# cherubicXN/neat

Hardware: AMD Instinct MI355X
Metric: ray-samples/s (train step) on ABC-neat-a (higher is better)
Workload: dtype bf16; 1 GPU; C2: abc-neat-a networks, 1024 rays x 128 samples per GPU, depth samples given, train step = forward + loss + backward + Adam; rays_per_gpu=1024, samples_per_ray=128, global_rays=1024, parallelism=dp1, weights=synthetic 'rough' (seed 42), launch=hip graph replay, the whole step one launch (forward + loss + backward + Adam)

## Files before the change

include/neat_hip.h:

```cpp
#ifndef NEAT_HIP_H
#define NEAT_HIP_H
#include <stddef.h>
#ifdef __cplusplus
extern "C" {
#endif

#define NEAT_NUM_LAYERS 19
#define NEAT_FEATURE 256

typedef struct neat_net_params {
  const float* v[NEAT_NUM_LAYERS];
  const float* g[NEAT_NUM_LAYERS];
  const float* b[NEAT_NUM_LAYERS];
} neat_net_params;

typedef struct neat_net_grads {
  float* dv[NEAT_NUM_LAYERS];
  float* dg[NEAT_NUM_LAYERS];
  float* db[NEAT_NUM_LAYERS];
} neat_net_grads;

int neat_abi_version(void);

#define NEAT_F32 0
// ... 129 lines not shown
int neat_project2d_pair(const float* K, const float* K2, const float* w2c, const float* X, int N, float* uv, float* uv2, void* stream);
int neat_line_loss(const float* pred, const float* gt, const float* weight, int R, float threshold, float* out2, float* per_line,
                   float* d_pred, void* stream);
int neat_line_losses(const float* pred_px, const float* pred_calib, const float* gt5, const float* K, int R, float threshold, float* out3,
                     float* d_pred_calib, float grad_scale, void* stream);

int neat_adam_step(float* params, const float* const* grads, const long long* seg_offsets, const int* seg_steps, int nseg,
                   float* exp_avg, float* exp_avg_sq, float lr, float beta1, float beta2, float eps, void* stream);
int neat_adam_step_coef(float* params, const float* const* grads, const long long* seg_offsets, int nseg, float* exp_avg, float* exp_avg_sq,
                        const float* coef, float beta1, float beta2, float eps, void* stream);

size_t neat_lsap_ws_bytes(int nr, int nc);
int neat_lsap(const float* cost, int nr, int nc, const unsigned char* row_mask, const unsigned char* col_mask, long long* row_ind,
              long long* col_ind, int* n_match, void* ws, void* stream);

size_t neat_dbscan_ws_bytes(int n);
int neat_dbscan_means(const float* points, int n, double eps, float* centres, unsigned char* valid, int* count, void* ws, void* stream);

int neat_parse_match(const float* lines2d, int n, const float* gt, int m, int gt_stride, float threshold, int* label, float* mindis,
                     void* stream);
size_t neat_parse_group_ws_bytes(int n, int m);
int neat_parse_group(const int* label, const float* lines3d, const float* l3d, int n, int m, float* lines, float* scores, int* count,
                     void* ws, void* stream);
size_t neat_parse_vote_ws_bytes(int J, int mcap);
int neat_parse_vote(const float* junctions, int J, const float* lines, const int* count, int mcap, float threshold, int view, int* votes,
                    int* first, void* ws, void* stream);
size_t neat_parse_graph_ws_bytes(int V, int mcap, int J);
int neat_parse_graph(const float* vlines, const float* vscores, const int* vcount, int V, int mcap, float score_threshold,
                     const float* junctions, const int* votes, const int* first, int J, float* lines_out, float* junc_out,
                     unsigned char* graph, int* pairs, float* wfi, int ecap, int* counts, void* ws, void* stream);
// ... 23 lines not shown
```

neat_amd/_lib.py:

```python
import ctypes
import os

NUM_LAYERS = 19
ABI_VERSION = 15
PRECISIONS = {"fp32": 0, "bf16": 1, "bf16x3": 2, "fp16": 3, "fp16x3": 4}
_HERE = os.path.dirname(os.path.abspath(__file__))
LIB_PATH = os.environ.get("NEAT_HIP_LIB") or os.path.join(_HERE, "csrc", "libneat_hip.so")

c_fp = ctypes.c_void_p


class NetParams(ctypes.Structure):
    _fields_ = [("v", c_fp * NUM_LAYERS), ("g", c_fp * NUM_LAYERS), ("b", c_fp * NUM_LAYERS)]


class NetGrads(ctypes.Structure):
    _fields_ = [("dv", c_fp * NUM_LAYERS), ("dg", c_fp * NUM_LAYERS), ("db", c_fp * NUM_LAYERS)]


_SIGNATURES = {
    "neat_abi_version": (ctypes.c_int, []),
    "neat_packed_floats": (ctypes.c_size_t, [ctypes.c_int]),
    "neat_pack_weights": (ctypes.c_int, [ctypes.POINTER(NetParams), c_fp, ctypes.c_int, c_fp]),
    "neat_eik_points": (ctypes.c_int, [c_fp, c_fp, c_fp, c_fp, c_fp, ctypes.c_int, ctypes.c_int, c_fp, c_fp, ctypes.c_int, c_fp, c_fp]),
# ... 65 lines not shown
                                          c_fp, c_fp, c_fp]),
    "neat_loss_terms": (ctypes.c_int, [c_fp, c_fp, ctypes.c_int, c_fp, ctypes.c_int, c_fp, c_fp, ctypes.c_int, c_fp, c_fp, ctypes.c_int,
                                       c_fp, c_fp, c_fp, c_fp, ctypes.c_float, c_fp]),
    "neat_loss_pairs": (ctypes.c_int, [c_fp, c_fp, c_fp, ctypes.c_int, c_fp, c_fp, c_fp, c_fp, c_fp, c_fp, ctypes.c_int, c_fp, c_fp, c_fp,
                                       c_fp, c_fp, ctypes.c_float, ctypes.c_float, ctypes.c_float, ctypes.c_float, ctypes.c_int, c_fp, c_fp, c_fp]),
    "neat_camera_mats": (ctypes.c_int, [c_fp, c_fp, ctypes.c_int, c_fp, c_fp, c_fp]),
    "neat_inv_small": (ctypes.c_int, [c_fp, ctypes.c_int, ctypes.c_int, c_fp, c_fp]),
    "neat_project2d": (ctypes.c_int, [c_fp, c_fp, c_fp, ctypes.c_int, c_fp, c_fp]),
    "neat_project2d_backward": (ctypes.c_int, [c_fp, c_fp, c_fp, ctypes.c_int, c_fp, c_fp, c_fp]),
    "neat_line_loss": (ctypes.c_int, [c_fp, c_fp, c_fp, ctypes.c_int, ctypes.c_float, c_fp, c_fp, c_fp, c_fp]),
    "neat_line_losses": (ctypes.c_int, [c_fp, c_fp, c_fp, c_fp, ctypes.c_int, ctypes.c_float, c_fp, c_fp, ctypes.c_float, c_fp]),
    "neat_adam_step": (ctypes.c_int, [c_fp, ctypes.POINTER(ctypes.c_void_p), ctypes.POINTER(ctypes.c_longlong), ctypes.POINTER(ctypes.c_int),
                                      ctypes.c_int, c_fp, c_fp, ctypes.c_float, ctypes.c_float, ctypes.c_float, ctypes.c_float, c_fp]),
    "neat_lsap_ws_bytes": (ctypes.c_size_t, [ctypes.c_int, ctypes.c_int]),
    "neat_lsap": (ctypes.c_int, [c_fp, ctypes.c_int, ctypes.c_int, c_fp, c_fp, c_fp, c_fp, c_fp, c_fp, c_fp]),
    "neat_dbscan_ws_bytes": (ctypes.c_size_t, [ctypes.c_int]),
    "neat_dbscan_means": (ctypes.c_int, [c_fp, ctypes.c_int, ctypes.c_double, c_fp, c_fp, c_fp, c_fp, c_fp]),
    "neat_parse_match": (ctypes.c_int, [c_fp, ctypes.c_int, c_fp, ctypes.c_int, ctypes.c_int, ctypes.c_float, c_fp, c_fp, c_fp]),
    "neat_parse_group_ws_bytes": (ctypes.c_size_t, [ctypes.c_int, ctypes.c_int]),
    "neat_parse_group": (ctypes.c_int, [c_fp, c_fp, c_fp, ctypes.c_int, ctypes.c_int, c_fp, c_fp, c_fp, c_fp, c_fp]),
    "neat_parse_vote_ws_bytes": (ctypes.c_size_t, [ctypes.c_int, ctypes.c_int]),
    "neat_parse_vote": (ctypes.c_int, [c_fp, ctypes.c_int, c_fp, c_fp, ctypes.c_int, ctypes.c_float, ctypes.c_int, c_fp, c_fp, c_fp, c_fp]),
    "neat_parse_graph_ws_bytes": (ctypes.c_size_t, [ctypes.c_int, ctypes.c_int, ctypes.c_int]),
    "neat_parse_graph": (ctypes.c_int, [c_fp, c_fp, c_fp, ctypes.c_int, ctypes.c_int, ctypes.c_float, c_fp, c_fp, c_fp, ctypes.c_int,
                                        c_fp, c_fp, c_fp, c_fp, c_fp, ctypes.c_int, c_fp, c_fp, c_fp]),
    "neat_parse_visibility_ws_bytes": (ctypes.c_size_t, [ctypes.c_int, ctypes.c_int]),
    "neat_parse_visibility": (ctypes.c_int, [c_fp, c_fp, ctypes.c_int, c_fp, ctypes.c_int, c_fp, c_fp, c_fp, ctypes.c_int, ctypes.c_float,
                                             ctypes.c_int, c_fp, c_fp, c_fp, c_fp, c_fp]),
    "neat_grid_points": (ctypes.c_int, [c_fp, ctypes.c_int, ctypes.c_longlong, ctypes.c_int, ctypes.POINTER(ctypes.c_int),
                                        ctypes.POINTER(ctypes.c_double), ctypes.POINTER(ctypes.c_double), c_fp]),
# ... 51 lines not shown
```

neat_amd/csrc/kernels_junction.hpp:

```cpp
#pragma once
#include <hip/hip_runtime.h>
#include "device_util.hpp"

namespace neat {

constexpr int LSAP_WG = 1024;

struct LsapArgs {
  const float* cost;
  int nr, nc;
  const unsigned char* row_mask;
  long long* row_ind;
  long long* col_ind;
  int* n_match;
  double* wsd;
  int* wsi;
  int use_lds, lds_int_off;
  const unsigned char* col_mask;
  int cost_lds_off;
};

struct LsapKey { double val; int it; int un; };

__device__ __forceinline__ bool lsap_better(const LsapKey& a, const LsapKey& b) {
// ... 1016 lines not shown
}

struct LossPairsArgs {
  const long long* ri; const long long* ci; const int* n_match; int Kmax;
  const float* loc3; const float* loc2c; const float* loc2;
  const float* glo3; const float* glo2c; const float* glo2; int J;
  const float* pair_cost;
  float* scal;
  float* d_glo3; float* d_glo2c;
  const float* line_loss; float w_eik, w_line, w_j3, w_j2;
  int weighted_grads;
  float* total;
  const float* w2c;
};

__global__ __launch_bounds__(1024) void loss_pairs_kernel(LossPairsArgs a) {
  __shared__ float s_red[16];
  const int tid = threadIdx.x, nt = blockDim.x;
  for (int i = tid; i < 3 * a.J; i += nt) a.d_glo3[i] = 0.0f;
  for (int i = tid; i < 2 * a.J; i += nt) a.d_glo2c[i] = 0.0f;
  __syncthreads();
  const int n = max(*a.n_match, 0);
  const float inv = 1.0f / (float)max(n, 1);
  const float g3 = a.weighted_grads ? a.w_j3 : 1.0f, g2 = a.weighted_grads ? a.w_j2 : 1.0f;
  float s3 = 0.0f, s2 = 0.0f, spx = 0.0f, cnt = 0.0f;
  for (int q = tid; q < a.Kmax; q += nt) {
    const long long r = a.ri[q], c = a.ci[q];
    if (r < 0 || c < 0 || q >= n) continue;
#pragma unroll
    for (int e = 0; e < 3; ++e) {
      const float d = a.loc3[3 * r + e] - a.glo3[3 * c + e];
// ... 15 lines not shown
      const float x[3] = {a.glo3[3 * j], a.glo3[3 * j + 1], a.glo3[3 * j + 2]};
      float dX[3];
      project_bwd_calib(a.w2c, x, a.d_glo2c[2 * j], a.d_glo2c[2 * j + 1], dX);
#pragma unroll
      for (int e = 0; e < 3; ++e) a.d_glo3[3 * j + e] += dX[e];
    }
  }
  if (tid == 0) {
    a.scal[2] = s3 * inv; a.scal[3] = s2 * inv; a.scal[4] = spx * inv; a.scal[5] = cnt;
    const float tot = a.scal[0] + a.w_eik * a.scal[1] + a.w_line * a.line_loss[0] + a.w_j3 * (s3 * inv) + a.w_j2 * (s2 * inv);
    a.scal[6] = tot;
    if (a.total) a.total[0] = tot;
  }
}

__global__ void l3d_kernel(const float* __restrict__ x, const float* __restrict__ o, const float* __restrict__ d,
                           const float* __restrict__ nrm, int R, float* __restrict__ l3d) {
  const int r = blockIdx.x * blockDim.x + threadIdx.x;
  if (r >= R) return;
  float den = 0.0f, num = 0.0f;
#pragma unroll
  for (int c = 0; c < 3; ++c) { den += d[3 * r + c] * nrm[3 * r + c]; num += (x[3 * r + c] - o[3 * r + c]) * nrm[3 * r + c]; }
  den += den >= 0.0f ? 1e-6f : -1e-6f;
  const float t = num / den;
#pragma unroll
  for (int c = 0; c < 3; ++c) l3d[3 * r + c] = o[3 * r + c] + d[3 * r + c] * t;
}

__global__ void junction_cost_kernel(const float* __restrict__ cand2d, const float* __restrict__ gt2d, int V, int C, float* __restrict__ cost) {
  const int idx = blockIdx.x * blockDim.x + threadIdx.x;
  if (idx >= V * C) return;
  const int v = idx / C, c = idx % C;
  const float dx = cand2d[2 * c] - gt2d[2 * v], dy = cand2d[2 * c + 1] - gt2d[2 * v + 1];
  cost[idx] = __fsqrt_rn(__fadd_rn(__fmul_rn(dx, dx), __fmul_rn(dy, dy)));
}

struct JunctionGateArgs {
  const long long* rows; const long long* cols; int K;
  const float* cost; int C;
  const float* cand3d; const float* cand2d; const float* cand2dc;
  int use_median;
  float* median;
  unsigned char* good;
  float* j3d; float* j2d; float* j2dc;
};

__global__ __launch_bounds__(1024) void junction_gate_kernel(JunctionGateArgs a) {
  __shared__ float s_m[2048];
  __shared__ int s_n;
  __shared__ float s_med;
  const int tid = threadIdx.x, nt = blockDim.x;
  if (tid == 0) { s_n = 0; s_med = 10.0f; }
  __syncthreads();
  for (int k = tid; k < a.K; k += nt) {
    const long long r = a.rows[k], c = a.cols[k];
    const bool ok = r >= 0 && c >= 0;
    s_m[k] = ok ? a.cost[r * a.C + c] : NAN;
    if (ok) atomicAdd(&s_n, 1);
  }
  __syncthreads();
  const int n = s_n;
  if (a.use_median && n > 0) {
// ... 9 lines not shown
  __syncthreads();
  const float thr = a.use_median ? s_med : 10.0f;
  if (tid == 0 && a.use_median) a.median[0] = s_med;
  for (int k = tid; k < a.K; k += nt) {
    const float v = s_m[k];
    const bool ok = v == v;
    a.good[k] = (ok && v < thr) ? 1 : 0;
    const long long c = ok ? a.cols[k] : 0;
#pragma unroll
    for (int e = 0; e < 3; ++e) a.j3d[3 * k + e] = ok ? a.cand3d[3 * c + e] : 0.0f;
#pragma unroll
    for (int e = 0; e < 2; ++e) { a.j2d[2 * k + e] = ok ? a.cand2d[2 * c + e] : 0.0f; a.j2dc[2 * k + e] = ok ? a.cand2dc[2 * c + e] : 0.0f; }
  }
}

}
```

neat_amd/csrc/neat_aux.hip:

```cpp
#include "kernels_sampler.hpp"
#include "kernels_junction.hpp"
#include "kernels_parse.hpp"
#include "kernels_mesh.hpp"
#include "../../include/neat_hip.h"
#include <algorithm>
#include <cmath>
#include <limits.h>
#include <math.h>

using namespace neat;

__attribute__((visibility("hidden"))) int neat_aux_set_tuning(int key, int value);

namespace {

int g_ffn_mfma = 1;
int g_sampler_ablate = 0;

#define NEAT_CHECK(expr) do { hipError_t e_ = (expr); if (e_ != hipSuccess) return (int)e_; } while (0)
inline dim3 grid1(int n, int b = 256) { return dim3((n + b - 1) / b); }

__global__ void volume_weights_kernel(const float* __restrict__ z, const float* __restrict__ sdf, int R, int S,
                                      const float* __restrict__ beta_ptr, float* __restrict__ weights) {
  const float beta = *beta_ptr;
// ... 439 lines not shown
  size_t lds = 0;
  constexpr size_t LSAP_LDS_MAX = 156 * 1024;
  a.cost_lds_off = -1;
  if (dbytes + ibytes <= LSAP_LDS_MAX) {
    NEAT_CHECK(lds_limit<&lsap_kernel>((int)LSAP_LDS_MAX));
    a.use_lds = 1; a.lds_int_off = (int)dbytes; lds = (dbytes + ibytes + 15) & ~(size_t)15;
    const size_t cbytes = (size_t)nr * nc * sizeof(float);
    if (lds + cbytes <= LSAP_LDS_MAX) { a.cost_lds_off = (int)lds; lds += cbytes; }
  }
  int threads = (int)((mx + 1) / 2 + 63) / 64 * 64;
  threads = threads < 64 ? 64 : (threads > LSAP_WG ? LSAP_WG : threads);
  hipLaunchKernelGGL(lsap_kernel, dim3(1), dim3(threads), lds, (hipStream_t)stream, a);
  return (int)hipGetLastError();
}

size_t neat_dbscan_ws_bytes(int n) { return (size_t)n * 2 * sizeof(int); }

int neat_dbscan_means(const float* points, int n, double eps, float* centres, unsigned char* valid, int* count, void* ws, void* stream) {
  if (n <= 0 || n > DBSCAN_MAXN || !points || !centres || !valid || !count || !ws || !(eps > 0.0)) return -1;
  int* parent = (int*)ws; int* has_nb = parent + n;
  hipLaunchKernelGGL(dbscan_init_kernel, dim3((n + 255) / 256), dim3(256), 0, (hipStream_t)stream, parent, has_nb, n);
  hipLaunchKernelGGL(dbscan_union_kernel, dim3(n), dim3(128), 0, (hipStream_t)stream, points, n, eps * eps, parent, has_nb);
  const size_t acc_bytes = (size_t)(n / 2) * 28 + (size_t)n * 4, pbytes = (size_t)n * 12;
  const int mode = acc_bytes <= 96 * 1024 ? 2 : (pbytes <= 96 * 1024 ? 1 : 0);
  if (mode) NEAT_CHECK(lds_limit<&dbscan_finish_kernel>(96 * 1024));
  hipLaunchKernelGGL(dbscan_finish_kernel, dim3(1), dim3(1024), mode == 2 ? acc_bytes : (mode == 1 ? pbytes : 0), (hipStream_t)stream, points, n,
                     parent, has_nb, centres, valid, count, mode);
  return (int)hipGetLastError();
}

// ... 200 lines not shown
```

neat_amd/networks.py:

```python
import math

import numpy as np
import os

import torch
from torch import nn

from . import ops, rend_util
from .conf import ConfTree, from_dict
from .density import LaplaceDensity
from .ray_sampler import ErrorBoundSampler, HierarchicalSampler


def _wn_linear(in_dim, out_dim, weight_norm=True):
    lin = nn.Linear(in_dim, out_dim)
    if not weight_norm:
        raise NotImplementedError("the HIP path implements the weight-normed layers of the shipped confs")
    return lin


DEFAULT_PRECISION = "fp16x3"


def _wrap_wn(lin):
# ... 390 lines not shown
        output = {"points": points, "rgb_values": rgb, "sdf": sdf_s, "depth": depth, "xyz": xyz}

        points3d = xyz
        main = torch.cuda.current_stream() if xyz.is_cuda else None
        side = self._side_stream(xyz.device) if (main is not None and self.use_side_stream) else None
        if setup is not None:
            w2c, K3 = setup[3], setup[4]
        elif xyz.is_cuda and pose.shape[1:] == (4, 4) and intrinsics.dtype == torch.float32 and intrinsics.stride(-1) == 1:
            w2c, K3 = ops.camera_mats(pose[0], intrinsics[0])
        else:
            w2c = ops.inv_small(pose[0])[:3]
            K3 = intrinsics[0, :3, :3]
        Rm, T = w2c[:, :3], w2c[:, 3:]
        eye = _eye3(K3.device)

        def l3d_block():
            if points3d.is_cuda:
                net = self.implicit_network
                p3_sdf, p3_grad = ops.sdf_point_normals(net.handle(), points3d, net.sdf_bounding_sphere, net.sphere_scale)
            else:
                p3_sdf, _, p3_grad = self.implicit_network.get_outputs(points3d)
            l_dirs, l_orig = (setup[2], cam_loc) if setup is not None else self._rays(input, "uv_proj")
            if points3d.is_cuda:
                l3d = ops.l3d_points(points3d, l_orig, l_dirs, p3_grad)
            else:
                den = (l_dirs * p3_grad).sum(-1)
                den = den + torch.where(den >= 0, torch.full_like(den, 1e-6), torch.full_like(den, -1e-6))
                t = (((points3d - l_orig) * p3_grad).sum(-1) / den).detach()
                l3d = l_orig + l_dirs * t.unsqueeze(-1)
            l3d_score = None
            if self.training and self.use_l3d:
                with torch.no_grad():
                    a, b = l3d - lines3d[:, 0], l3d - lines3d[:, 1]
                    l3d_score = torch.linalg.cross(a, b).norm(dim=-1) / (lines3d[:, 0] - lines3d[:, 1]).norm(dim=-1)
            return p3_sdf, l3d, l3d_score

        j3d_global = None
        if side is not None:
# ... 21 lines not shown
                side_b = None
        else:
            side_b = None
            if self.training:
                j3d_global = self._global_junctions()
            p3_sdf, l3d, l3d_score = l3d_block()
        if xyz.is_cuda:
            K3c, w2c3 = K3.contiguous(), w2c.contiguous()
            K3 = K3c
            proj = lambda Kc, X: ops.project2d(Kc, w2c3, X)
            proj_pair = lambda X: ops.project2d_pair(K3c, eye, w2c3, X)
        else:
            K3c = K3
            proj = lambda Kc, X: self.project2D(Kc, Rm, T, X)
            proj_pair = lambda X: (proj(K3c, X), proj(eye, X))
        if xyz.is_cuda:
            lines2d, lines2d_calib = proj_pair(lines3d)
            lines2d = lines2d.detach()
        else:
            lines2d = proj(K3c, lines3d.detach())
            lines2d_calib = proj(eye, lines3d)
        if self.training:
            cand_valid = None
            if self.dbscan_enabled:
                if lines3d.is_cuda and 2 <= 2 * n_rays <= ops.DBSCAN_MAX_POINTS:
                    cand3d, cand_valid, _ = ops.dbscan_means(lines3d.detach().reshape(-1, 3), 0.01)
                else:
                    cand3d = self.cluster_dbscan(lines3d.detach().cpu().numpy().reshape(-1, 3), eps=0.01, min_samples=2)
            elif self.use_l3d:
                thr = l3d_score.median().clamp_min(0.01)
                keep = l3d_score < thr
                cand3d = torch.cat([lines3d[keep].detach().reshape(-1, 3), l3d[keep]], 0)
            else:
                cand3d = lines3d.detach().reshape(-1, 3)
            if self.dbscan_enabled or self.use_l3d:
                cand2d, cand2d_calib = proj_pair(cand3d)
            else:
                cand2d = lines2d.reshape(-1, 2)
                cand2d_calib = lines2d_calib.detach().reshape(-1, 2)
            gt2d = _device_copy(input["wireframe"][0], "vertices", cand2d.device)
            fused_gate = cand2d.is_cuda and min(gt2d.shape[0], cand2d.shape[0]) <= 2048
            cost = ops.junction_cost(cand2d, gt2d) if fused_gate else ((cand2d[None] - gt2d[:, None]) ** 2).sum(-1).sqrt()
            rows, cols, _ = ops.linear_sum_assignment(cost, None, cand_valid)
            if fused_gate:
                median, good, j3_pad, j2_pad, j2c_pad = ops.junction_gate(rows, cols, cost, cand3d, cand2d, cand2d_calib, self.use_median)
                if self.use_median:
                    output["median"] = median
            else:
                if cand_valid is None:
                    matched = cost[rows, cols]
                    pair_ok = None
                else:
                    pair_ok = rows >= 0
                    rows, cols = rows.clamp_min(0), cols.clamp_min(0)
                    matched = torch.where(pair_ok, cost[rows, cols], torch.full_like(cost[rows, cols], float("nan")))
# ... 85 lines not shown
```

neat_amd/ops.py:

```python
import ctypes

import torch

from . import _lib

NET_LAYOUT = (("implicit_network", 9), ("rendering_network", 5), ("attraction_network", 5))
LAYER_OUT = [256, 256, 256, 217, 256, 256, 256, 256, 257, 256, 256, 256, 256, 3, 256, 256, 256, 256, 6]
LAYER_IN = [39, 256, 256, 256, 256, 256, 256, 256, 256, 289, 256, 256, 256, 256, 265, 256, 256, 256, 256]
N_SDF = 9


def _p(t):
    return ctypes.c_void_p(t.data_ptr()) if t is not None else None


def _stream():
    return ctypes.c_void_p(torch.cuda.current_stream().cuda_stream)


def copy_batch(pairs):
    lib = _lib.lib()
    for i0 in range(0, len(pairs), 16):
        chunk = pairs[i0:i0 + 16]
        n = len(chunk)
# ... 748 lines not shown
        line3 = torch.empty(3, device=dev)
        fold = lines3d is not None and w2c is not None
        x3_c, w2c_c = (_f32c(lines3d.detach().reshape(-1, 6)), _f32c(w2c.detach())) if fold else (None, None)
        if fold and (x3_c.shape[0] != L or w2c_c.shape != (3, 4)):
            raise RuntimeError("loss_tail: lines3d [L,2,3] and w2c [3,4]")
        sizes = [R * 3, E * 3, J * 3 if have_pairs else 0, J * 2 if have_pairs else 0, L * 4, L * 6 if fold else 0]
        flat = torch.empty(sum(sizes), device=dev)
        d_rgb, d_gth, d_glo3, d_glo2c, d_pred, d_x3 = flat.split(sizes)
        d_gth = d_gth if E else None
        pair_cost = torch.empty(K, J, device=dev) if have_pairs else None
        _lib.check(lib.neat_loss_lines_terms(_p(pu), _p(pc), _p(g5), _p(Kc), L, float(threshold), _p(line3), _p(d_pred), w_line,
                                             _p(rgb_c), _p(gt_c), R, _p(gth_c), E, _p(loc3_c), _p(loc2c_c), K, _p(glo3_c), _p(glo2c_c), J,
                                             _p(scal), _p(d_rgb), _p(d_gth), _p(pair_cost), w_eik, _p(w2c_c), _p(x3_c), _p(d_x3) if fold else None,
                                             _stream()), "neat_loss_lines_terms")
        if have_pairs:
            ri, ci, n_match = linear_sum_assignment(pair_cost, good)
            loss = torch.empty((), device=dev)
            _lib.check(lib.neat_loss_pairs(_p(ri), _p(ci), _p(n_match), ri.shape[0], _p(loc3_c), _p(loc2c_c), _p(loc2_c), _p(glo3_c),
                                           _p(glo2c_c), _p(glo2_c), J, _p(pair_cost), _p(scal), _p(d_glo3), _p(d_glo2c),
                                           _ip(line3, 1), w_eik, w_line, w_j3, w_j2, 1, _p(loss), _p(w2c_c), _stream()), "neat_loss_pairs")
        else:
            loss = scal[0] + w_eik * scal[1] + w_line * line3[1]
        ctx.save_for_backward(flat)
        ctx.sizes = sizes
        ctx.set_materialize_grads(False)
        ctx.shapes = (rgb.shape, None if gtheta is None else gtheta.shape, None if glo3 is None or not have_pairs else glo3.shape,
                      None if glo2c is None or not have_pairs or fold else glo2c.shape, None if fold else pred_calib.shape,
                      lines3d.shape if fold else None)
        ctx.mark_non_differentiable(scal, line3)
        return loss, scal, line3

    @staticmethod
    def backward(ctx, g_loss, g_scal, g_line3):
        if g_loss is None:
            return (None,) * 21
# ... 124 lines not shown
    _lib.check(_lib.lib().neat_junction_cost(_p(cand2d), _p(gt2d), V, C, _p(cost), _stream()), "neat_junction_cost")
    return cost


def junction_gate(rows, cols, cost, cand3d, cand2d, cand2d_calib, use_median):
    K = rows.shape[0]
    dev = cost.device
    cand3d, cand2d, cand2d_calib = _f32c(cand3d.detach()), _f32c(cand2d.detach()), _f32c(cand2d_calib.detach())
    median = torch.empty(1, device=dev) if use_median else None
    good = torch.empty(K, device=dev, dtype=torch.uint8)
    j3d, j2d, j2dc = torch.empty(K, 3, device=dev), torch.empty(K, 2, device=dev), torch.empty(K, 2, device=dev)
    _lib.check(_lib.lib().neat_junction_gate(_p(rows), _p(cols), K, _p(cost), cost.shape[1], _p(cand3d), _p(cand2d), _p(cand2d_calib),
                                             1 if use_median else 0, _p(median), _p(good), _p(j3d), _p(j2d), _p(j2dc), _stream()),
               "neat_junction_gate")
    return (median.reshape(()) if use_median else None), good.view(torch.bool), j3d, j2d, j2dc


def _i32(t):
    if t.dtype != torch.int32 or not t.is_cuda:
        raise RuntimeError("neat_amd parse ops need CUDA int32 tensors: got %s on %s" % (t.dtype, t.device))
    return t.contiguous()


def _ws(nbytes, device):
    return torch.empty(max(int(nbytes), 8), device=device, dtype=torch.uint8)


def _rows4(gt):
    gt = _f32c(gt.detach()) if gt.stride(-1) != 1 or gt.dtype != torch.float32 or not gt.is_cuda else gt.detach()
    if gt.dim() != 2 or gt.shape[1] < 4:
# ... 118 lines not shown
```

Baseline: 49.27 million ray-samples/s.

## Fuse junction projection, cost, LSAP and gating into single-wave GPU kernels

Adds a wave-level Hungarian (LSAP) solver for small assignment problems and fuses it with the projection, cost-matrix build and junction gating into one kernel. Extra blocks of the same launch also compute l3d and the global junction projections. A second fused kernel runs the pair LSAP inside the loss-pairs kernel. The aim is to cut the chain of small kernel launches and the separate general LSAP path inside the graphed train step. In exchange it adds LDS-bound size limits and a serial single-wave solver that only covers small problem sizes.

```diff
diff --git a/include/neat_hip.h b/include/neat_hip.h
--- a/include/neat_hip.h
+++ b/include/neat_hip.h
@@ -167,6 +167,17 @@
 int neat_lsap(const float* cost, int nr, int nc, const unsigned char* row_mask, const unsigned char* col_mask, long long* row_ind,
               long long* col_ind, int* n_match, void* ws, void* stream);
 
+int neat_lsap_few_ok(int nr, int nc);
+int neat_junction_match(const float* K, const float* K2, const float* w2c, const float* cand3d, int C, const unsigned char* cand_valid,
+                        const float* gt2d, int V, int use_median, float* cand2d, float* cand2d_calib, long long* rows, long long* cols,
+                        int* n_match, float* median, unsigned char* good, float* j3d, float* j2d, float* j2d_calib, const float* l_x,
+                        const float* l_o, const float* l_d, const float* l_normal, int R, float* l3d, const float* glo3, int J, float* glo2,
+                        float* glo2_calib, void* stream);
+int neat_loss_pairs_match(const float* pair_cost, int K, int J, const unsigned char* good, long long* ri, long long* ci, int* n_match,
+                          const float* loc3, const float* loc2c, const float* loc2, const float* glo3, const float* glo2c, const float* glo2,
+                          float* scal, float* d_glo3, float* d_glo2c, const float* line_loss, float w_eik, float w_line, float w_j3, float w_j2,
+                          int weighted_grads, float* total, const float* w2c, void* stream);
+
 size_t neat_dbscan_ws_bytes(int n);
 int neat_dbscan_means(const float* points, int n, double eps, float* centres, unsigned char* valid, int* count, void* ws, void* stream);
 
diff --git a/neat_amd/_lib.py b/neat_amd/_lib.py
--- a/neat_amd/_lib.py
+++ b/neat_amd/_lib.py
@@ -103,6 +103,11 @@
                                       ctypes.c_int, c_fp, c_fp, ctypes.c_float, ctypes.c_float, ctypes.c_float, ctypes.c_float, c_fp]),
     "neat_lsap_ws_bytes": (ctypes.c_size_t, [ctypes.c_int, ctypes.c_int]),
     "neat_lsap": (ctypes.c_int, [c_fp, ctypes.c_int, ctypes.c_int, c_fp, c_fp, c_fp, c_fp, c_fp, c_fp, c_fp]),
+    "neat_lsap_few_ok": (ctypes.c_int, [ctypes.c_int, ctypes.c_int]),
+    "neat_junction_match": (ctypes.c_int, [c_fp, c_fp, c_fp, c_fp, ctypes.c_int, c_fp, c_fp, ctypes.c_int, ctypes.c_int] + [c_fp] * 14
+                            + [ctypes.c_int, c_fp, c_fp, ctypes.c_int, c_fp, c_fp, c_fp]),
+    "neat_loss_pairs_match": (ctypes.c_int, [c_fp, ctypes.c_int, ctypes.c_int] + [c_fp] * 14
+                              + [ctypes.c_float, ctypes.c_float, ctypes.c_float, ctypes.c_float, ctypes.c_int, c_fp, c_fp, c_fp]),
     "neat_dbscan_ws_bytes": (ctypes.c_size_t, [ctypes.c_int]),
     "neat_dbscan_means": (ctypes.c_int, [c_fp, ctypes.c_int, ctypes.c_double, c_fp, c_fp, c_fp, c_fp, c_fp]),
     "neat_parse_match": (ctypes.c_int, [c_fp, ctypes.c_int, c_fp, ctypes.c_int, ctypes.c_int, ctypes.c_float, c_fp, c_fp, c_fp]),
diff --git a/neat_amd/csrc/kernels_junction.hpp b/neat_amd/csrc/kernels_junction.hpp
--- a/neat_amd/csrc/kernels_junction.hpp
+++ b/neat_amd/csrc/kernels_junction.hpp
@@ -1054,7 +1054,7 @@
   const float* w2c;
 };
 
-__global__ __launch_bounds__(1024) void loss_pairs_kernel(LossPairsArgs a) {
+__device__ __forceinline__ void loss_pairs_body(const LossPairsArgs& a) {
   __shared__ float s_red[16];
   const int tid = threadIdx.x, nt = blockDim.x;
   for (int i = tid; i < 3 * a.J; i += nt) a.d_glo3[i] = 0.0f;
@@ -1100,25 +1100,38 @@
   }
 }
 
+__global__ __launch_bounds__(1024) void loss_pairs_kernel(LossPairsArgs a) { loss_pairs_body(a); }
+
+__device__ __forceinline__ void l3d_point(const float* __restrict__ x, const float* __restrict__ o, const float* __restrict__ d,
+                                          const float* __restrict__ nrm, int r, float* __restrict__ l3d) {
+  float den = 0.0f, num = 0.0f;
+#pragma unroll
+  for (int c = 0; c < 3; ++c) { den += d[3 * r + c] * nrm[3 * r + c]; num += (x[3 * r + c] - o[3 * r + c]) * nrm[3 * r + c]; }
+  den += den >= 0.0f ? 1e-6f : -1e-6f;
+  const float t = num / den;
+#pragma unroll
+  for (int c = 0; c < 3; ++c) l3d[3 * r + c] = o[3 * r + c] + d[3 * r + c] * t;
+}
+
 __global__ void l3d_kernel(const float* __restrict__ x, const float* __restrict__ o, const float* __restrict__ d,
                            const float* __restrict__ nrm, int R, float* __restrict__ l3d) {
   const int r = blockIdx.x * blockDim.x + threadIdx.x;
   if (r >= R) return;
-  float den = 0.0f, num = 0.0f;
-#pragma unroll
-  for (int c = 0; c < 3; ++c) { den += d[3 * r + c] * nrm[3 * r + c]; num += (x[3 * r + c] - o[3 * r + c]) * nrm[3 * r + c]; }
-  den += den >= 0.0f ? 1e-6f : -1e-6f;
-  const float t = num / den;
-#pragma unroll
-  for (int c = 0; c < 3; ++c) l3d[3 * r + c] = o[3 * r + c] + d[3 * r + c] * t;
+  l3d_point(x, o, d, nrm, r, l3d);
+}
+
+__device__ __forceinline__ float junction_cost_value(float cx, float cy, float gx, float gy) {
+  const float dx = cx - gx, dy = cy - gy;
+  float xx = __fmul_rn(dx, dx), yy = __fmul_rn(dy, dy);
+  asm volatile("" : "+v"(xx), "+v"(yy));
+  return __fsqrt_rn(__fadd_rn(xx, yy));
 }
 
 __global__ void junction_cost_kernel(const float* __restrict__ cand2d, const float* __restrict__ gt2d, int V, int C, float* __restrict__ cost) {
   const int idx = blockIdx.x * blockDim.x + threadIdx.x;
   if (idx >= V * C) return;
   const int v = idx / C, c = idx % C;
-  const float dx = cand2d[2 * c] - gt2d[2 * v], dy = cand2d[2 * c + 1] - gt2d[2 * v + 1];
-  cost[idx] = __fsqrt_rn(__fadd_rn(__fmul_rn(dx, dx), __fmul_rn(dy, dy)));
+  cost[idx] = junction_cost_value(cand2d[2 * c], cand2d[2 * c + 1], gt2d[2 * v], gt2d[2 * v + 1]);
 }
 
 struct JunctionGateArgs {
@@ -1131,7 +1144,7 @@
   float* j3d; float* j2d; float* j2dc;
 };
 
-__global__ __launch_bounds__(1024) void junction_gate_kernel(JunctionGateArgs a) {
+__device__ __forceinline__ void junction_gate_body(const JunctionGateArgs& a) {
   __shared__ float s_m[2048];
   __shared__ int s_n;
   __shared__ float s_med;
@@ -1171,4 +1184,210 @@
   }
 }
 
-}
+__global__ __launch_bounds__(1024) void junction_gate_kernel(JunctionGateArgs a) { junction_gate_body(a); }
+
+constexpr int LSAP_FEW_MAXN = 32, LSAP_FEW_MAXM = 2048, LSAP_FEW_MAXCOST = 16384;
+
+__host__ __device__ inline bool lsap_few_ok(int nr, int nc) {
+  const int mn = nr < nc ? nr : nc, mx = nr < nc ? nc : nr;
+  return mn >= 1 && mn <= LSAP_FEW_MAXN && mx <= LSAP_FEW_MAXM && (long long)nr * nc <= LSAP_FEW_MAXCOST;
+}
+__host__ __device__ inline size_t lsap_few_work_bytes(int nr, int nc) {
+  const size_t mn = (size_t)(nr < nc ? nr : nc), mx = (size_t)(nr < nc ? nc : nr);
+  return (mn + 2 * mx) * sizeof(double) + ((size_t)nr + (size_t)nc + 3 * mx + 3 * mn) * sizeof(int);
+}
+__host__ __device__ inline size_t lsap_few_cost_bytes(int nr, int nc) { return ((size_t)nr * nc * sizeof(float) + 15) & ~(size_t)15; }
+
+__device__ __forceinline__ void wave_lds_sync() {
+  __builtin_amdgcn_fence(__ATOMIC_RELEASE, "wavefront");
+  __builtin_amdgcn_wave_barrier();
+  __builtin_amdgcn_fence(__ATOMIC_ACQUIRE, "wavefront");
+}
+
+template <class F>
+__device__ __forceinline__ int wave_compact(int n, F flag, int* out) {
+  const int lane = threadIdx.x & 63;
+  int base = 0;
+  for (int b0 = 0; b0 < n; b0 += 64) {
+    const int i = b0 + lane;
+    const bool f = i < n && flag(i);
+    const unsigned long long bal = __ballot(f);
+    if (f) out[base + __popcll(bal & ((1ull << lane) - 1ull))] = i;
+    base += __popcll(bal);
+  }
+  return base;
+}
+
+template <class CF>
+__device__ void lsap_few_wave(int nr, int nc, const unsigned char* mask, const unsigned char* cmask, CF C, unsigned char* work,
+                              long long* row_ind, long long* col_ind, int* n_match) {
+  const int lane = threadIdx.x & 63;
+  const int kmax = min(nr, nc), mx = max(nr, nc);
+  for (int k = lane; k < kmax; k += 64) { row_ind[k] = -1; col_ind[k] = -1; }
+  double* wsd = reinterpret_cast<double*>(work);
+  int* rowlist = reinterpret_cast<int*>(wsd + kmax + 2 * mx);
+  int* collist = rowlist + nr;
+  int n_eff, c_eff;
+  const bool ident = !mask && !cmask;
+  if (ident) { n_eff = nr; c_eff = nc; }
+  else {
+    n_eff = wave_compact(nr, [&](int i) { return mask ? mask[i] != 0 : true; }, rowlist);
+    c_eff = wave_compact(nc, [&](int j) { return cmask ? cmask[j] != 0 : true; }, collist);
+  }
+  const bool T = c_eff < n_eff;
+  const int N = T ? c_eff : n_eff, M = T ? n_eff : c_eff;
+  if (N == 0) { if (lane == 0) *n_match = 0; return; }
+  double* u = wsd; double* v = u + N; double* sp = v + M;
+  int* path = collist + nc; int* col4row = path + M; int* row4col = col4row + N; int* remaining = row4col + M;
+  int* vis_row = remaining + M;
+  int* vis_col = vis_row + N;
+  for (int i = lane; i < N; i += 64) { u[i] = 0.0; col4row[i] = -1; }
+  for (int j = lane; j < M; j += 64) { v[j] = 0.0; row4col[j] = -1; }
+  wave_lds_sync();
+  auto cost = [&](int i, int j) -> double {
+    return (double)(ident ? (T ? C(j, i) : C(i, j)) : (T ? C(rowlist[j], collist[i]) : C(rowlist[i], collist[j])));
+  };
+  bool fail = false;
+  for (int cur = 0; cur < N && !fail; ++cur) {
+    int i = cur, nrem = M, nvis = 0;
+    double minval = 0.0;
+    bool first = true;
+    while (true) {
+      const double ui = u[i];
+      LsapKey best{INFINITY, -1, 0};
+      if (first) {
+        for (int it = lane; it < M; it += 64) {
+          const int j = M - 1 - it;
+          const double r = minval + cost(i, j) - ui - v[j];
+          const bool lower = r < INFINITY;
+          const double spj = lower ? r : INFINITY;
+          sp[j] = spj;
+          if (lower) path[j] = i;
+          remaining[it] = j;
+          LsapKey k{spj, it, row4col[j] == -1 ? 1 : 0};
+          if (spj < INFINITY && lsap_better(k, best)) best = k;
+        }
+        first = false;
+      } else {
+        for (int it = lane; it < nrem; it += 64) {
+          const int j = remaining[it];
+          const double r = minval + cost(i, j) - ui - v[j];
+          double spj = sp[j];
+          if (r < spj) { path[j] = i; sp[j] = r; spj = r; }
+          LsapKey k{spj, it, row4col[j] == -1 ? 1 : 0};
+          if (spj < INFINITY && lsap_better(k, best)) best = k;
+        }
+      }
+      for (int m = 32; m >= 1; m >>= 1) {
+        LsapKey o = lsap_shfl_xor(best, m);
+        if (lsap_better(o, best)) best = o;
+      }
+      wave_lds_sync();
+      if (best.it < 0) { fail = true; break; }
+      const double mv = best.val;
+      const int j = remaining[best.it];
+      const int last = remaining[nrem - 1];
+      const int r4 = row4col[j];
+      wave_lds_sync();
+      if (lane == 0) { vis_row[nvis] = i; vis_col[nvis] = j; remaining[best.it] = last; }
+      ++nvis;
+      if (r4 != -1) { i = r4; minval = mv; nrem -= 1; wave_lds_sync(); continue; }
+      if (lane == 0) {
+        for (int q = 0; q < nvis; ++q) {
+          const int r_ = vis_row[q];
+          if (r_ == cur) u[r_] += mv;
+          else u[r_] += mv - sp[col4row[r_]];
+        }
+        for (int q = 0; q < nvis; ++q) { const int c_ = vis_col[q]; v[c_] -= mv - sp[c_]; }
+        int jj = j;
+        while (true) {
+          const int ii = path[jj];
+          row4col[jj] = ii;
+          const int t = col4row[ii]; col4row[ii] = jj; jj = t;
+          if (ii == cur) break;
+        }
+      }
+      wave_lds_sync();
+      break;
+    }
+  }
+  if (fail) { if (lane == 0) *n_match = -1; return; }
+  if (!T) {
+    for (int i = lane; i < N; i += 64) { row_ind[i] = ident ? i : rowlist[i]; col_ind[i] = ident ? col4row[i] : collist[col4row[i]]; }
+  } else {
+    int* tmp = remaining;
+    const int cnt = wave_compact(M, [&](int k) { return row4col[k] != -1; }, tmp);
+    wave_lds_sync();
+    for (int q = lane; q < cnt; q += 64) {
+      const int k = tmp[q];
+      row_ind[q] = ident ? k : rowlist[k]; col_ind[q] = ident ? row4col[k] : collist[row4col[k]];
+    }
+  }
+  if (lane == 0) *n_match = N;
+}
+
+struct JunctionMatchArgs {
+  const float* K; const float* K2; const float* w2c;
+  const float* cand3d; int C; const unsigned char* cand_valid;
+  const float* gt2d; int V;
+  float* cand2d; float* cand2dc;
+  long long* rows; long long* cols; int* n_match;
+  JunctionGateArgs gate;
+  const float* l_x; const float* l_o; const float* l_d; const float* l_n; int R; float* l3d; int l3d_blocks;
+  const float* glo3; int J; float* glo2; float* glo2c;
+};
+
+__device__ __forceinline__ void project2d_pair_point(const float* K, const float* K2, const float* w2c, const float* X, int i, float* uv, float* uv2) {
+  const float x[3] = {X[3 * i], X[3 * i + 1], X[3 * i + 2]};
+  float cam[3], w;
+  project_point(K, w2c, x, cam, w);
+  uv[2 * i] = cam[0] / w; uv[2 * i + 1] = cam[1] / w;
+  project_point(K2, w2c, x, cam, w);
+  uv2[2 * i] = cam[0] / w; uv2[2 * i + 1] = cam[1] / w;
+}
+
+__global__ __launch_bounds__(1024) void junction_match_kernel(JunctionMatchArgs a) {
+  extern __shared__ __attribute__((aligned(16))) unsigned char jm_lds[];
+  const int tid = threadIdx.x, nt = blockDim.x;
+  if (blockIdx.x > 0) {
+    const int b = blockIdx.x - 1;
+    if (b < a.l3d_blocks) {
+      const int r = b * nt + tid;
+      if (r < a.R) l3d_point(a.l_x, a.l_o, a.l_d, a.l_n, r, a.l3d);
+    } else {
+      const int j = (b - a.l3d_blocks) * nt + tid;
+      if (j < a.J) project2d_pair_point(a.K, a.K2, a.w2c, a.glo3, j, a.glo2, a.glo2c);
+    }
+    return;
+  }
+  float* s_cost = reinterpret_cast<float*>(jm_lds);
+  const int C = a.C, V = a.V;
+  for (int c = tid; c < C; c += nt) {
+    project2d_pair_point(a.K, a.K2, a.w2c, a.cand3d, c, a.cand2d, a.cand2dc);
+    const float cx = a.cand2d[2 * c], cy = a.cand2d[2 * c + 1];
+    for (int v = 0; v < V; ++v) s_cost[v * C + c] = junction_cost_value(cx, cy, a.gt2d[2 * v], a.gt2d[2 * v + 1]);
+  }
+  __syncthreads();
+  if (tid < 64)
+    lsap_few_wave(V, C, nullptr, a.cand_valid, [&](int r, int c) { return s_cost[r * C + c]; }, jm_lds + lsap_few_cost_bytes(V, C),
+                  a.rows, a.cols, a.n_match);
+  __syncthreads();
+  JunctionGateArgs g = a.gate;
+  g.rows = a.rows; g.cols = a.cols; g.K = min(V, C); g.cost = s_cost; g.C = C; g.cand3d = a.cand3d; g.cand2d = a.cand2d; g.cand2dc = a.cand2dc;
+  junction_gate_body(g);
+}
+
+__global__ __launch_bounds__(1024) void loss_pairs_match_kernel(LossPairsArgs a, int K, const unsigned char* good, long long* ri, long long* ci,
+                                                                int* n_match) {
+  extern __shared__ __attribute__((aligned(16))) unsigned char lpm_lds[];
+  const int tid = threadIdx.x, nt = blockDim.x, J = a.J;
+  float* s_cost = reinterpret_cast<float*>(lpm_lds);
+  for (int e = tid; e < K * J; e += nt) s_cost[e] = a.pair_cost[e];
+  __syncthreads();
+  if (tid < 64)
+    lsap_few_wave(K, J, good, nullptr, [&](int r, int c) { return s_cost[r * J + c]; }, lpm_lds + lsap_few_cost_bytes(K, J), ri, ci, n_match);
+  __syncthreads();
+  loss_pairs_body(a);
+}
+
+}
diff --git a/neat_amd/csrc/neat_aux.hip b/neat_amd/csrc/neat_aux.hip
--- a/neat_amd/csrc/neat_aux.hip
+++ b/neat_amd/csrc/neat_aux.hip
@@ -477,6 +477,42 @@
   return (int)hipGetLastError();
 }
 
+int neat_lsap_few_ok(int nr, int nc) { return lsap_few_ok(nr, nc) ? 1 : 0; }
+
+int neat_junction_match(const float* K, const float* K2, const float* w2c, const float* cand3d, int C, const unsigned char* cand_valid,
+                        const float* gt2d, int V, int use_median, float* cand2d, float* cand2d_calib, long long* rows, long long* cols,
+                        int* n_match, float* median, unsigned char* good, float* j3d, float* j2d, float* j2d_calib, const float* l_x,
+                        const float* l_o, const float* l_d, const float* l_normal, int R, float* l3d, const float* glo3, int J, float* glo2,
+                        float* glo2_calib, void* stream) {
+  if (!lsap_few_ok(V, C) || R < 0 || J < 0) return -1;
+  if (!K || !K2 || !w2c || !cand3d || !gt2d || !cand2d || !cand2d_calib || !rows || !cols || !n_match || !good || !j3d || !j2d || !j2d_calib ||
+      (use_median && !median) || (R > 0 && (!l_x || !l_o || !l_d || !l_normal || !l3d)) || (J > 0 && (!glo3 || !glo2 || !glo2_calib))) return -1;
+  JunctionMatchArgs a{};
+  a.K = K; a.K2 = K2; a.w2c = w2c; a.cand3d = cand3d; a.C = C; a.cand_valid = cand_valid; a.gt2d = gt2d; a.V = V;
+  a.cand2d = cand2d; a.cand2dc = cand2d_calib; a.rows = rows; a.cols = cols; a.n_match = n_match;
+  a.gate.use_median = use_median; a.gate.median = median; a.gate.good = good; a.gate.j3d = j3d; a.gate.j2d = j2d; a.gate.j2dc = j2d_calib;
+  a.l_x = l_x; a.l_o = l_o; a.l_d = l_d; a.l_n = l_normal; a.R = R; a.l3d = l3d; a.l3d_blocks = (R + 1023) / 1024;
+  a.glo3 = glo3; a.J = J; a.glo2 = glo2; a.glo2c = glo2_calib;
+  const size_t lds = lsap_few_cost_bytes(V, C) + lsap_few_work_bytes(V, C);
+  NEAT_CHECK(lds_limit<&junction_match_kernel>((int)lds));
+  hipLaunchKernelGGL(junction_match_kernel, dim3(1 + a.l3d_blocks + (J + 1023) / 1024), dim3(1024), lds, (hipStream_t)stream, a);
+  return (int)hipGetLastError();
+}
+
+int neat_loss_pairs_match(const float* pair_cost, int K, int J, const unsigned char* good, long long* ri, long long* ci, int* n_match,
+                          const float* loc3, const float* loc2c, const float* loc2, const float* glo3, const float* glo2c, const float* glo2,
+                          float* scal, float* d_glo3, float* d_glo2c, const float* line_loss, float w_eik, float w_line, float w_j3, float w_j2,
+                          int weighted_grads, float* total, const float* w2c, void* stream) {
+  if (!lsap_few_ok(K, J) || !ri || !ci || !n_match || !loc3 || !loc2c || !loc2 || !glo3 || !glo2c || !glo2 || !pair_cost || !scal ||
+      !d_glo3 || !d_glo2c || !line_loss) return -1;
+  LossPairsArgs a{ri, ci, n_match, K < J ? K : J, loc3, loc2c, loc2, glo3, glo2c, glo2, J, pair_cost, scal, d_glo3, d_glo2c, line_loss, w_eik, w_line,
+                  w_j3, w_j2, weighted_grads, total, w2c};
+  const size_t lds = lsap_few_cost_bytes(K, J) + lsap_few_work_bytes(K, J);
+  NEAT_CHECK(lds_limit<&loss_pairs_match_kernel>((int)lds));
+  hipLaunchKernelGGL(loss_pairs_match_kernel, dim3(1), dim3(1024), lds, (hipStream_t)stream, a, K, good, ri, ci, n_match);
+  return (int)hipGetLastError();
+}
+
 size_t neat_dbscan_ws_bytes(int n) { return (size_t)n * 2 * sizeof(int); }
 
 int neat_dbscan_means(const float* points, int n, double eps, float* centres, unsigned char* valid, int* count, void* ws, void* stream) {
diff --git a/neat_amd/networks.py b/neat_amd/networks.py
--- a/neat_amd/networks.py
+++ b/neat_amd/networks.py
@@ -428,6 +428,15 @@
         Rm, T = w2c[:, :3], w2c[:, 3:]
         eye = _eye3(K3.device)
 
+        gt2d = None
+        fused_match = False
+        if self.training and xyz.is_cuda and side is None and not self.use_l3d:
+            gt2d = _device_copy(input["wireframe"][0], "vertices", xyz.device)
+            n_cand = n_rays if self.dbscan_enabled else 2 * n_rays
+            fused_match = (gt2d.dim() == 2 and gt2d.shape[1] == 2 and (not self.dbscan_enabled or 2 <= 2 * n_rays <= ops.DBSCAN_MAX_POINTS)
+                           and ops.junction_fused_ok(gt2d.shape[0], n_cand))
+        l3d_pending = []
+
         def l3d_block():
             if points3d.is_cuda:
                 net = self.implicit_network
@@ -435,7 +444,10 @@
             else:
                 p3_sdf, _, p3_grad = self.implicit_network.get_outputs(points3d)
             l_dirs, l_orig = (setup[2], cam_loc) if setup is not None else self._rays(input, "uv_proj")
-            if points3d.is_cuda:
+            if fused_match:
+                l3d_pending.append((points3d, l_orig, l_dirs, p3_grad))
+                l3d = None
+            elif points3d.is_cuda:
                 l3d = ops.l3d_points(points3d, l_orig, l_dirs, p3_grad)
             else:
                 den = (l_dirs * p3_grad).sum(-1)
@@ -487,13 +499,33 @@
             K3c = K3
             proj = lambda Kc, X: self.project2D(Kc, Rm, T, X)
             proj_pair = lambda X: (proj(K3c, X), proj(eye, X))
-        if xyz.is_cuda:
+        fm = None
+        if fused_match:
+            if self.dbscan_enabled:
+                lines2d, lines2d_calib = proj_pair(lines3d)
+                lines2d = lines2d.detach()
+                cand3d, cand_valid, _ = ops.dbscan_means(lines3d.detach().reshape(-1, 3), 0.01)
+                fm = ops.junction_match(K3c, eye, w2c3, cand3d, cand_valid, gt2d, self.use_median, l3d_pending[0], j3d_global)
+            else:
+                fm = ops.junction_match(K3c, eye, w2c3, lines3d, None, gt2d, self.use_median, l3d_pending[0], j3d_global)
+                lines2d, lines2d_calib = fm[0], fm[1]
+            l3d = fm[10]
+        elif xyz.is_cuda:
             lines2d, lines2d_calib = proj_pair(lines3d)
             lines2d = lines2d.detach()
         else:
             lines2d = proj(K3c, lines3d.detach())
             lines2d_calib = proj(eye, lines3d)
-        if self.training:
+        if fm is not None:
+            median, good, j3_pad, j2_pad, j2c_pad = fm[5], fm[6], fm[7], fm[8], fm[9]
+            if self.use_median:
+                output["median"] = median
+            output = JunctionOutputs(output, good, {"j2d_local": j2_pad, "j3d_local": j3_pad, "j2d_local_calib": j2c_pad})
+            output["j3d_global"] = j3d_global
+            output["j2d_global"], output["j2d_global_calib"] = fm[11], fm[12]
+            output.calib_proj = {"w2c": w2c3, "lines3d": lines3d, "lines2d_calib": lines2d_calib, "j3d_global": j3d_global,
+                                 "j2d_global_calib": output["j2d_global_calib"]}
+        elif self.training:
             cand_valid = None
             if self.dbscan_enabled:
                 if lines3d.is_cuda and 2 <= 2 * n_rays <= ops.DBSCAN_MAX_POINTS:
@@ -511,7 +543,8 @@
             else:
                 cand2d = lines2d.reshape(-1, 2)
                 cand2d_calib = lines2d_calib.detach().reshape(-1, 2)
-            gt2d = _device_copy(input["wireframe"][0], "vertices", cand2d.device)
+            if gt2d is None:
+                gt2d = _device_copy(input["wireframe"][0], "vertices", cand2d.device)
             fused_gate = cand2d.is_cuda and min(gt2d.shape[0], cand2d.shape[0]) <= 2048
             cost = ops.junction_cost(cand2d, gt2d) if fused_gate else ((cand2d[None] - gt2d[:, None]) ** 2).sum(-1).sqrt()
             rows, cols, _ = ops.linear_sum_assignment(cost, None, cand_valid)
diff --git a/neat_amd/ops.py b/neat_amd/ops.py
--- a/neat_amd/ops.py
+++ b/neat_amd/ops.py
@@ -786,11 +786,20 @@
                                              _p(scal), _p(d_rgb), _p(d_gth), _p(pair_cost), w_eik, _p(w2c_c), _p(x3_c), _p(d_x3) if fold else None,
                                              _stream()), "neat_loss_lines_terms")
         if have_pairs:
-            ri, ci, n_match = linear_sum_assignment(pair_cost, good)
             loss = torch.empty((), device=dev)
-            _lib.check(lib.neat_loss_pairs(_p(ri), _p(ci), _p(n_match), ri.shape[0], _p(loc3_c), _p(loc2c_c), _p(loc2_c), _p(glo3_c),
-                                           _p(glo2c_c), _p(glo2_c), J, _p(pair_cost), _p(scal), _p(d_glo3), _p(d_glo2c),
-                                           _ip(line3, 1), w_eik, w_line, w_j3, w_j2, 1, _p(loss), _p(w2c_c), _stream()), "neat_loss_pairs")
+            if junction_fused_ok(K, J):
+                kk = min(K, J)
+                ri, ci = torch.empty(kk, device=dev, dtype=torch.int64), torch.empty(kk, device=dev, dtype=torch.int64)
+                n_match = torch.empty(1, device=dev, dtype=torch.int32)
+                _lib.check(lib.neat_loss_pairs_match(_p(pair_cost), K, J, _p(_as_u8(good)), _p(ri), _p(ci), _p(n_match), _p(loc3_c), _p(loc2c_c),
+                                                     _p(loc2_c), _p(glo3_c), _p(glo2c_c), _p(glo2_c), _p(scal), _p(d_glo3), _p(d_glo2c),
+                                                     _ip(line3, 1), w_eik, w_line, w_j3, w_j2, 1, _p(loss), _p(w2c_c), _stream()),
+                           "neat_loss_pairs_match")
+            else:
+                ri, ci, n_match = linear_sum_assignment(pair_cost, good)
+                _lib.check(lib.neat_loss_pairs(_p(ri), _p(ci), _p(n_match), ri.shape[0], _p(loc3_c), _p(loc2c_c), _p(loc2_c), _p(glo3_c),
+                                               _p(glo2c_c), _p(glo2_c), J, _p(pair_cost), _p(scal), _p(d_glo3), _p(d_glo2c),
+                                               _ip(line3, 1), w_eik, w_line, w_j3, w_j2, 1, _p(loss), _p(w2c_c), _stream()), "neat_loss_pairs")
         else:
             loss = scal[0] + w_eik * scal[1] + w_line * line3[1]
         ctx.save_for_backward(flat)
@@ -945,6 +954,91 @@
                                              1 if use_median else 0, _p(median), _p(good), _p(j3d), _p(j2d), _p(j2dc), _stream()),
                "neat_junction_gate")
     return (median.reshape(()) if use_median else None), good.view(torch.bool), j3d, j2d, j2dc
+
+
+_JUNCTION_FUSED = [True]
+
+
+class junction_fused:
+
+    def __init__(self, enabled):
+        self.enabled = bool(enabled)
+
+    def __enter__(self):
+        self.prev, _JUNCTION_FUSED[0] = _JUNCTION_FUSED[0], self.enabled
+        return self
+
+    def __exit__(self, *exc):
+        _JUNCTION_FUSED[0] = self.prev
+        return False
+
+
+def junction_fused_ok(nr, nc):
+    return bool(_JUNCTION_FUSED[0] and _lib.lib().neat_lsap_few_ok(int(nr), int(nc)))
+
+
+class JunctionMatchFn(torch.autograd.Function):
+
+    @staticmethod
+    def forward(ctx, K3, K3b, w2c, X, cand_valid, gt2d, use_median, l_x, l_o, l_d, l_n, glo3):
+        lib = _lib.lib()
+        K3, K3b, w2c = _f32c(K3.detach()), _f32c(K3b.detach()), _f32c(w2c.detach())
+        Xc, gt = _f32c(X.detach().reshape(-1, 3)), _f32c(gt2d.detach())
+        dev = Xc.device
+        C, V = Xc.shape[0], gt.shape[0]
+        if not lib.neat_lsap_few_ok(V, C):
+            raise RuntimeError("junction_match: %d x %d is outside the few-row path (ops.junction_fused_ok)" % (V, C))
+        k = min(V, C)
+        uv, uv2 = torch.empty(C, 2, device=dev), torch.empty(C, 2, device=dev)
+        rows, cols = torch.empty(k, device=dev, dtype=torch.int64), torch.empty(k, device=dev, dtype=torch.int64)
+        n_match = torch.empty(1, device=dev, dtype=torch.int32)
+        median = torch.empty(1, device=dev) if use_median else None
+        good = torch.empty(k, device=dev, dtype=torch.uint8)
+        j3d, j2d, j2dc = torch.empty(k, 3, device=dev), torch.empty(k, 2, device=dev), torch.empty(k, 2, device=dev)
+        R = 0 if l_x is None else l_x.shape[0]
+        lin = [None if t is None else _f32c(t.detach().reshape(-1, 3)) for t in (l_x, l_o, l_d, l_n)]
+        l3d = torch.empty(R, 3, device=dev) if R else None
+        Gc = None if glo3 is None else _f32c(glo3.detach().reshape(-1, 3))
+        J = 0 if Gc is None else Gc.shape[0]
+        g2, g2c = (torch.empty(J, 2, device=dev), torch.empty(J, 2, device=dev)) if J else (None, None)
+        _lib.check(lib.neat_junction_match(_p(K3), _p(K3b), _p(w2c), _p(Xc), C, _p(_as_u8(cand_valid)), _p(gt), V, 1 if use_median else 0,
+                                           _p(uv), _p(uv2), _p(rows), _p(cols), _p(n_match), _p(median), _p(good), _p(j3d), _p(j2d), _p(j2dc),
+                                           _p(lin[0]), _p(lin[1]), _p(lin[2]), _p(lin[3]), R, _p(l3d), _p(Gc), J, _p(g2), _p(g2c), _stream()),
+                   "neat_junction_match")
+        ctx.save_for_backward(K3, K3b, w2c, Xc, Gc)
+        ctx.shape, ctx.gshape = X.shape, None if glo3 is None else glo3.shape
+        ctx.set_materialize_grads(False)
+        uv, uv2 = uv.reshape(*X.shape[:-1], 2), uv2.reshape(*X.shape[:-1], 2)
+        if J:
+            g2, g2c = g2.reshape(*glo3.shape[:-1], 2), g2c.reshape(*glo3.shape[:-1], 2)
+        good = good.view(torch.bool)
+        med = median.reshape(()) if use_median else None
+        ctx.mark_non_differentiable(*[t for t in (uv, rows, cols, n_match, med, good, j3d, j2d, j2dc, l3d) if t is not None])
+        return uv, uv2, rows, cols, n_match, med, good, j3d, j2d, j2dc, l3d, g2, g2c
+
+    @staticmethod
+    def backward(ctx, d_uv, d_uv2, d_rows, d_cols, d_n, d_med, d_good, d_j3, d_j2, d_j2c, d_l3d, d_g2, d_g2c):
+        K3, K3b, w2c, Xc, Gc = ctx.saved_tensors
+
+        def back(P, pairs, shape):
+            total = None
+            for Kx, d in pairs:
+                if d is None:
+                    continue
+                dX = torch.empty_like(P)
+                _lib.check(_lib.lib().neat_project2d_backward(_p(Kx), _p(w2c), _p(P), P.shape[0], _p(_f32c(d.reshape(-1, 2))), _p(dX), _stream()),
+                           "neat_project2d_backward")
+                total = dX if total is None else total + dX
+            return None if total is None else total.reshape(shape)
+
+        dX = back(Xc, ((K3b, d_uv2),), ctx.shape)
+        dG = back(Gc, ((K3, d_g2), (K3b, d_g2c)), ctx.gshape) if Gc is not None else None
+        return None, None, None, dX, None, None, None, None, None, None, None, dG
+
+
+def junction_match(K3, K3b, w2c, X, cand_valid, gt2d, use_median, l3d_inputs=None, glo3=None):
+    lx, lo, ld, ln = l3d_inputs if l3d_inputs is not None else (None, None, None, None)
+    return JunctionMatchFn.apply(K3, K3b, w2c, X, cand_valid, gt2d, bool(use_median), lx, lo, ld, ln, glo3)
 
 
 def _i32(t):
```

New measurement: 43.45 million ray-samples/s. -11.8%, worse.
